# HyperBitGore/deflate.hpp

Hardware: AMD Instinct MI355X
Metric: GB/s deflate+inflate on 1 GiB buffer at 1/2/4/8 MI355X; ratio vs reference (higher is better)
Workload: dtype u8; 1 GPU; deflate level 2 + inflate round trip of a per-GPU 1 GiB 'repeat' corpus (SURVEY App. B), device-resident; corpus=repeat, bytes_per_gpu=1073741824, level=2, segment_bytes=32768, parallelism=shard1

## Files before the change

deflate.hpp_amd/csrc/deflate_kernels.hip:

```cpp
#include "dmx_device.h"
#include "dmx_internal.h"

namespace dmx {

constexpr int DF_NT = 1024;
constexpr int DF_CHUNK = 258;
constexpr int df_hash_bits(int seg) {
    return seg >= 32768 ? 12 : 11;
}
constexpr int DF_LIT_MAXBITS = 9;
constexpr int DF_DIST_MAXBITS = 6;
constexpr int DF_L3_DEPTH = 16;
constexpr uint32_t DF_L3_LONG = 16;
constexpr uint32_t DF_L3_RP = 512;
constexpr bool df_early(int seg) { return seg >= 32768; }
constexpr uint32_t EM_ALL_LITERALS = 0xFFFFFFFFu;


__device__ __forceinline__ int df_tid() {
    int t = threadIdx.x;
    asm volatile("" : "+v"(t));
    return t;
}

// ... 318 lines not shown
            const uint64_t d = *B.nseg_dev;
            return d < A.nseg ? d : A.nseg;
        }
    }
    return A.nseg;
}

template <int SEG, bool BATCH, bool DICT = false>
__device__ __forceinline__ DfSegAddr df_seg_addr(const DeflateArgs& A, uint64_t seg) {
    static_assert(!DICT || BATCH, "the dictionary comes with the batch's segment table");
    DfSegAddr s;
    s.dict = nullptr;
    s.dlen = 0;
    if constexpr (BATCH) {
        const DeflateBatchSeg e = A.btab[seg];
        s.src = e.src;
        s.tail = e.tail;
        s.nb = e.nb;
        s.is_last = (e.buf & DF_BATCH_LAST) != 0;
        if constexpr (DICT) {
            s.dict = e.dict;
            s.dlen = (uint32_t)e.dlen;
        }
    } else {
        const uint64_t base = seg * (uint64_t)SEG;
        s.src = A.in + base;
        s.tail = A.n - base;
        s.nb = (uint32_t)min((uint64_t)SEG, A.n - base);
        s.is_last = seg + 1 == A.nseg;
    }
    return s;
}

template <int SEG, bool BATCH, bool DICT = false>
__device__ __forceinline__ bool df_prefetch_next(const DeflateArgs& A, uint64_t seg, uint32_t* image) {
    bool go;
    const uint8_t* nsrc;
    if constexpr (BATCH) {
        go = seg + gridDim.x < df_nseg<true>(A);
        if (go) {
            const DeflateBatchSeg e = A.btab[seg + gridDim.x];
            nsrc = e.src;
            go = e.nb == (uint32_t)SEG && ((reinterpret_cast<uintptr_t>(nsrc) & 15) == 0);
            if constexpr (DICT) go = go && e.dlen == 0;
        } else {
            nsrc = nullptr;
        }
    } else {
        const uint64_t nbase = (seg + gridDim.x) * (uint64_t)SEG;
        nsrc = A.in + nbase;
        go = seg + gridDim.x < A.nseg && nbase + SEG <= A.n && ((reinterpret_cast<uintptr_t>(A.in + nbase) & 15) == 0);
    }
    if (go) {
        const int t = df_tid();
        const uint4* src = reinterpret_cast<const uint4*>(nsrc) + t;
        uint4* dst = reinterpret_cast<uint4*>(image) + (t & ~63);
        if constexpr (df_early(SEG)) {
            static_assert(4 * DfSmem<SEG>::NWALK <= DF_NT / 2, "the walk leaves the upper waves idle");
            if (t >= DF_NT / 2) {
                const uint32_t base = __builtin_amdgcn_readfirstlane(
                    (uint32_t)(uintptr_t)(__attribute__((address_space(3))) void*)(dst - DF_NT / 2));
#pragma unroll
                for (int k = 0; k < SEG / (8 * DF_NT); k++) {
                    uint32_t keep;
                    asm volatile("s_mov_b32 %0, m0\n\ts_mov_b32 m0, %2\n\ts_nop 0\n\t"
                                 "global_load_lds_dwordx4 %1, off\n\ts_mov_b32 m0, %0"
                                 : "=&s"(keep)
                                 : "v"(src - DF_NT / 2 + k * (DF_NT / 2)), "s"(base + (uint32_t)(k * DF_NT * 8))
                                 : "memory");
                }
            }
        } else {
#pragma unroll
            for (int k = 0; k < SEG / (16 * DF_NT); k++)
                __builtin_amdgcn_global_load_lds(src + k * DF_NT, (__attribute__((address_space(3))) void*)(dst + k * DF_NT),
                                                 16, 0, 0);
        }
    }
    return go;
}

struct TokRange {
    uint32_t w, m, n;
};
__device__ __forceinline__ uint32_t next_tok(const uint32_t* tokmap, uint32_t& w, uint32_t& m) {
    while (!m) m = tokmap[++w];
    const uint32_t p = w * 32 + __builtin_ctz(m);
    m &= m - 1;
    return p;
}

__device__ __forceinline__ void df_load_at(uint8_t* dbytes, uint32_t off, const uint8_t* src, uint32_t n, int t) {
    uint32_t head = (16u - (off & 15u)) & 15u;
    if (((reinterpret_cast<uintptr_t>(src) + head) & 15) != 0 || head > n) head = n;
    for (uint32_t i = t; i < head; i += DF_NT) dbytes[off + i] = src[i];
    const uint32_t nvec = (n - head) / 16;
    const uint4* s4 = reinterpret_cast<const uint4*>(src + head);
    uint4* d4 = reinterpret_cast<uint4*>(dbytes + off + head);
    for (uint32_t i = t; i < nvec; i += DF_NT) d4[i] = s4[i];
    for (uint32_t i = head + 16 * nvec + t; i < n; i += DF_NT) dbytes[off + i] = src[i];
}

template <int SEG, bool L3, bool BATCH, bool DICT>
__device__ __forceinline__ void deflate_segment(const DeflateArgs& A, DfSmem<SEG>& S, uint64_t seg,
                                                uint32_t& staged, [[maybe_unused]] uint32_t iw) {
    constexpr bool EARLY = DfSmem<SEG>::EARLY;
    uint32_t *data32, *U;
    if constexpr (EARLY) {
        data32 = &S.buf[0][0] + iw;
        U = &S.buf[0][0] + ((uint32_t)DfSmem<SEG>::BW - iw);
    } else {
        data32 = S.data32;
        U = S.U;
    }
    [[maybe_unused]] constexpr int NWALK = DfSmem<SEG>::NWALK;
    constexpr int HT = DfSmem<SEG>::HT;
    constexpr int NMAP = SEG / 32;
    const int t = df_tid();
    const DfSegAddr sa = df_seg_addr<SEG, BATCH, DICT>(A, seg);
    const uint32_t D = DICT ? sa.dlen : 0u;
    const uint32_t nb = D + sa.nb;
    constexpr int level = L3 ? 3 : 2;
    uint8_t* const dbytes = reinterpret_cast<uint8_t*>(data32);
    constexpr bool TERMRUN = !L3 && SEG >= 32768;
    constexpr uint32_t RUN_NONE = 0xFFFFFFFFu;
    DMX_PHASE(A.dbg, seg, 0);

    {
        const uint8_t* src = sa.src;
        const uint32_t nvec = nb / 16;
        if (staged) {
        } else if (DICT && D) {
            df_load_at(dbytes, 0, sa.dict, D, t);
            df_load_at(dbytes, D, src, nb - D, t);
        } else if ((((uintptr_t)src) & 15) == 0) {
            const uint4* s4 = reinterpret_cast<const uint4*>(src);
// ... 254 lines not shown
                    for (int j = 0; j < 4; j++) {
                        m |= ((x[j] & 0xFFFFu) ? 1u : 0u) << (8 * k + 2 * j);
                        m |= ((x[j] >> 16) ? 1u : 0u) << (8 * k + 2 * j + 1);
                    }
                }
                const uint32_t b0 = 32 * w;
                S.mmap[w] = b0 + 32 <= nb ? m : (nb > b0 ? m & ((1u << (nb - b0)) - 1u) : 0u);
            }
            if (TERMRUN && run_lo != RUN_NONE) {
                const uint32_t v = run_d | (run_d << 16);
                const uint32_t i0 = run_lo / 8, i1 = max(i0, (nb - 11) / 8 + 1);
                uint4* const c4 = reinterpret_cast<uint4*>(S.cand);
                for (uint32_t i = i0 + t; i < i1; i += DF_NT) c4[i] = make_uint4(v, v, v, v);
                const uint32_t p = 8 * i1 + t;
                if (t < 16 && p < nb) S.cand[p] = (uint16_t)(p + 4 <= nb ? run_d : 0u);
                constexpr uint32_t RP = 2 * DF_NT;
                const uint32_t bq = run_lo - RP + 4 * (uint32_t)t;
                if ((uint32_t)t < RP / 4 && bq >= run_d) {
                    const uint32_t ia = (bq - run_d) >> 2;
                    const uint32_t df = data32[bq >> 2] ^
                                        __builtin_amdgcn_alignbyte(data32[ia + 1], data32[ia], (run_lo - run_d) & 3);
                    if (df) atomicMax(&S.sh[43], ((run_lo / RP + 1) << 16) | (bq + 4 - ((uint32_t)__builtin_clz(df) >> 3)));
                }
            }
            __syncthreads();
            if (TERMRUN && run_lo != RUN_NONE) {
                constexpr uint32_t RP = 2 * DF_NT;
                const uint32_t et = __builtin_amdgcn_readfirstlane(S.sh[43]);
                run_e = (et >> 16) == run_lo / RP + 1 ? et & 0xFFFFu : max(run_lo - RP, (run_d + 3) & ~3u);
                run_rcp = __builtin_amdgcn_rcpf((float)run_d);
            }
        }
        DMX_PHASE(A.dbg, seg, 2);
        if constexpr (EARLY) staged = df_prefetch_next<SEG, BATCH, DICT>(A, seg, U);

        constexpr uint32_t CH = DF_CHUNK;
        const uint32_t nwalk = (nb - D + CH - 1) / CH;
        auto parse_walk = [&](auto runc) {
            constexpr bool RUNW = decltype(runc)::value;
            const uint32_t sub = t & 3;
            const bool lead = sub == 0;
            const uint32_t lo = D + (t >> 2) * CH;
            const uint32_t hi = min(lo + CH, nb);
            auto bits_range = [](uint32_t a, uint32_t b, uint32_t w) -> uint32_t {
                const uint32_t e = b - w * 32;
                return (e >= 32 ? 0xFFFFFFFFu : ((1u << e) - 1u)) & (0xFFFFFFFFu << (a & 31));
            };
            [[maybe_unused]] auto known_len = [&](uint32_t q, uint32_t d) -> bool {
                const uint32_t m = (uint32_t)((float)d * run_rcp + 0.5f);
                return (q >= run_e) & (m * run_d == d) & (q - d + run_d >= run_e);
            };
            auto len_at = [&](uint32_t q, uint32_t d, uint32_t maxl) -> uint32_t {
                if (!RUNW) return matchlen4(data32, q, q - d, maxl, sub);
                const bool kn = known_len(q, d);
                const uint32_t L = matchlen4(data32, q, q - d, kn ? 0u : maxl, sub);
                return kn ? maxl : L;
            };
            auto full_len = [&](uint32_t q) -> uint32_t {
                return len_at(q, S.cand[q], min(258u, hi - q));
            };
            uint32_t p = lo, w = lo >> 5, mw = S.mmap[w], tok = 0, lastp = lo;
            auto mbit = [&](uint32_t q) -> bool {
                return (S.mmap[q >> 5] >> (q & 31)) & 1u;
            };
            while (p < hi) {
                const uint32_t wi = p >> 5;
                if (wi != w) {
// ... 284 lines not shown
                    uint32_t w = tr.w, m = tr.m, lit = 0, nl = 0;
                    for (uint32_t i = 0; i < tr.n; i++) {
                        const uint32_t p = next_tok(S.tokmap, w, m);
                        const uint32_t d = S.cand[p];
                        if (d) {
                            if (nl) emit(lit | (nl << 24));
                            nl = 0;
                            lit = 0;
                            emit(0x80000000u | ((uint32_t)(S.cand[p + 1] - 3) << 16) | (d - 1));
                        } else {
                            lit |= (uint32_t)data_byte(data32, p) << (8 * nl);
                            if (++nl == 3) {
                                emit(lit | (3u << 24));
                                nl = 0;
                                lit = 0;
                            }
                        }
                    }
                    if (nl) emit(lit | (nl << 24));
                };
                uint32_t nw = 0;
                walk([&](uint32_t) { nw++; });
                uint32_t wtot;
                const uint32_t woff = block_excl_scan(nw, S.scan, &wtot);
                uint32_t* const dst = A.tok + seg * (uint64_t)A.tok_stride + woff;
                uint32_t j = 0;
                walk([&](uint32_t v) { dst[j++] = v; });
                if (t == 0) A.ntok[seg] = wtot;
            }
        }
        DMX_PHASE(A.dbg, seg, 11);
        if constexpr (!EARLY) {
            __syncthreads();
            staged = df_prefetch_next<SEG, BATCH, DICT>(A, seg, data32);
        }
        DMX_PHASE(A.dbg, seg, 10);
    }
}

template <int SEG, bool L3, bool BATCH, bool DICT>
__device__ __forceinline__ void deflate_segments(const DeflateArgs& A, DfSmem<SEG>& S) {
    constexpr bool EARLY = DfSmem<SEG>::EARLY;
    uint32_t staged = 0;
    uint32_t iw = 0;
    if constexpr (EARLY) {
        const int t = df_tid();
        if (t < 64) S.buf[t >> 5][SEG / 4 + (t & 31)] = 0;
    }
    for (uint64_t seg = blockIdx.x; seg < df_nseg<BATCH>(A); seg += gridDim.x) {
        deflate_segment<SEG, L3, BATCH, DICT>(A, S, seg, staged, iw);
        if constexpr (EARLY) {
            df_lds_barrier();
            iw = (uint32_t)DfSmem<SEG>::BW - iw;
        } else
            __syncthreads();
    }
}
template <int SEG, bool L3, bool BATCH = false, bool DICT = false>
__global__ __launch_bounds__(DF_NT) void k_deflate_segments(DeflateArgs A) {
    static_assert(!BATCH && !DICT, "a batch runs k_deflate_segments_batch");
    __shared__ DfSmem<SEG> S;
    deflate_segments<SEG, L3, false, false>(A, S);
}
template <bool L3, bool BATCH = false>
__global__ __launch_bounds__(DF_NT) __attribute__((amdgpu_waves_per_eu(8, 8))) void k_deflate_segments16(DeflateArgs A) {
    static_assert(!BATCH, "a batch runs k_deflate_segments16_batch");
    __shared__ DfSmem<16384> S;
    deflate_segments<16384, L3, false, false>(A, S);
}
template <int SEG, bool L3, bool DICT = false>
__global__ __launch_bounds__(DF_NT) void k_deflate_segments_batch(DeflateBatchArgs A) {
    __shared__ DfSmem<SEG> S;
    deflate_segments<SEG, L3, true, DICT>(A, S);
}
template <bool L3>
__global__ __launch_bounds__(DF_NT) __attribute__((amdgpu_waves_per_eu(8, 8))) void k_deflate_segments16_batch(DeflateBatchArgs A) {
    __shared__ DfSmem<16384> S;
    deflate_segments<16384, L3, true, false>(A, S);
}

constexpr int EM_NW = 4;
constexpr int EM_FLUSH = 256;
constexpr int EM_STG = 576;
constexpr int EM_LIT = 288, EM_SYM = 320;

struct EmWave {
    union {
        uint32_t freq[EM_SYM];
        uint32_t stg[EM_STG];
    };
    uint32_t code[EM_SYM];
    uint8_t len[EM_SYM];
    uint16_t rk[EM_SYM];
    uint32_t prefreq[20];
    uint32_t precode[20];
    uint8_t prelen[24];
    uint32_t hcnt[6][20];
    uint32_t lcnt[6][16];
    uint32_t kpre[2][20];
    uint32_t start[2][16];
    uint32_t next[2][16];
};

struct EmCodes {
    uint32_t dyn_tok, fix_tok;
    uint32_t nlit, ndist;
};

__device__ __forceinline__ uint32_t em_slot(int c, int lane) { return c < 5 ? 64 * c + lane : EM_LIT + lane; }
__device__ __forceinline__ bool em_valid(int c, int lane) { return c < 5 ? 64 * c + lane < 286 : lane < 30; }

__device__ EmCodes em_build_codes(EmWave& W) {
    const int lane = lane_id();
    const uint64_t lt = (1ull << lane) - 1ull;
    uint32_t Fl = 0, nzl = 0, hil = 0;
    for (int c = 0; c < 5; c++) {
        const uint32_t f = em_valid(c, lane) ? W.freq[em_slot(c, lane)] : 0u;
        Fl += f;
        const uint64_t b = __ballot(f != 0);
        nzl += (uint32_t)__popcll(b);
        if (b) hil = 64 * c + 64 - (uint32_t)__clzll(b);
    }
    Fl = wave_sum(Fl);
    const uint32_t f5 = lane < 30 ? W.freq[EM_LIT + lane] : 0u;
    const uint32_t Fd = wave_sum(f5);
    const uint64_t bd = __ballot(f5 != 0);
    const uint32_t nzd = (uint32_t)__popcll(bd), hid = bd ? 64 - (uint32_t)__clzll(bd) : 0u;
    for (int c = 0; c < 6; c++) {
        const uint32_t f = em_valid(c, lane) ? W.freq[em_slot(c, lane)] : 0u;
        const uint32_t F = c < 5 ? Fl : Fd;
        const uint32_t L0 = init_len(f, F, c < 5 ? DF_LIT_MAXBITS : DF_DIST_MAXBITS);
        const uint32_t k0 = L0 ? 2 * L0 + (((uint64_t)f << L0) <= F ? 1u : 0u) : 0u;
        uint32_t mine = 0, w0 = 0;
#pragma unroll
        for (int k = 2; k <= 2 * DF_LIT_MAXBITS + 1; k++) {
// ... 468 lines not shown
        }
        return w;
    };
#pragma unroll 4
    for (uint32_t k4 = lane; k4 < n16; k4 += 64) {
        uint4 o;
        if (const uint32_t sh = data_shift(16 * k4, 16 * k4 + 16)) {
            const uint32_t x = 16 * k4 - sh + mis, i0 = x >> 2, s = x & 3;
            const uint32_t a0 = inw[i0], a1 = inw[i0 + 1], a2 = inw[i0 + 2], a3 = inw[i0 + 3];
            const uint32_t a4 = i0 + 4 < in_words_end ? inw[i0 + 4] : 0u;
            o.x = __builtin_amdgcn_alignbyte(a1, a0, s);
            o.y = __builtin_amdgcn_alignbyte(a2, a1, s);
            o.z = __builtin_amdgcn_alignbyte(a3, a2, s);
            o.w = __builtin_amdgcn_alignbyte(a4, a3, s);
        } else {
            o.x = word_at(4 * k4);
            o.y = word_at(4 * k4 + 1);
            o.z = word_at(4 * k4 + 2);
            o.w = word_at(4 * k4 + 3);
        }
        slot4[k4] = o;
    }
    if (lane == 0) A.sizes[seg] = total;
}

template <int SEG, bool RAW, bool BATCH = false>
__global__ __launch_bounds__(64 * EM_NW) __attribute__((amdgpu_waves_per_eu(6))) void k_deflate_emit(DeflateArgs A) {
    static_assert(!BATCH, "a batch runs k_deflate_emit_batch");
    __shared__ EmWave Ws[EM_NW];
    const uint64_t seg = (uint64_t)blockIdx.x * EM_NW + (threadIdx.x >> 6);
    if (seg >= A.nseg) return;
    em_segment<SEG, RAW, false>(A, Ws[threadIdx.x >> 6], seg);
}
template <int SEG, bool RAW>
__global__ __launch_bounds__(64 * EM_NW) __attribute__((amdgpu_waves_per_eu(6))) void k_deflate_emit_batch(DeflateBatchArgs A) {
    __shared__ EmWave Ws[EM_NW];
    const uint64_t seg = (uint64_t)blockIdx.x * EM_NW + (threadIdx.x >> 6);
    if (seg >= df_nseg<true>(A)) return;
    em_segment<SEG, RAW, true>(A, Ws[threadIdx.x >> 6], seg);
}

constexpr uint32_t SCAN_NT = 256, SCAN_PER = 32, SCAN_BLK = SCAN_NT * SCAN_PER;
__device__ __forceinline__ void scan_load32(const uint32_t* v, uint64_t i, uint64_t n, bool vec, uint32_t (&x)[32]) {
    if (vec && i + 32 <= n) {
        const uint4* s4 = reinterpret_cast<const uint4*>(v + i);
#pragma unroll
        for (int k = 0; k < 8; k++) {
            const uint4 q = s4[k];
            x[4 * k] = q.x;
            x[4 * k + 1] = q.y;
            x[4 * k + 2] = q.z;
            x[4 * k + 3] = q.w;
        }
    } else {
#pragma unroll
        for (int k = 0; k < 32; k++) x[k] = i + k < n ? v[i + k] : 0u;
    }
}
__device__ __forceinline__ uint64_t scan_block64(uint64_t s, uint64_t* part, uint64_t* all) {
    const int t = threadIdx.x, lane = t & 63, wave = t >> 6;
    uint64_t inc = s;
#pragma unroll
    for (int d = 1; d < 64; d <<= 1) {
        const uint32_t lo = (uint32_t)__shfl_up((int)(uint32_t)inc, d, 64);
        const uint32_t hi = (uint32_t)__shfl_up((int)(uint32_t)(inc >> 32), d, 64);
        if (lane >= d) inc += ((uint64_t)hi << 32) | lo;
// ... 111 lines not shown
        r.path = 0;
        A.bres[b] = r;
        return;
    }
    const uint64_t s0 = A.bfirst[b], s1 = A.bfirst[b + 1];
    uint64_t bytes;
    if (s0 == s1) {
        bytes = 2;
        if (A.bcap[b] >= 2) {
            A.bout[b][0] = 0x03;
            A.bout[b][1] = 0x00;
        }
    } else {
        bytes = (s1 < A.nseg ? A.offsets[s1] : *A.total) - A.offsets[s0];
    }
    ::dmx_batch_result r;
    r.bytes = bytes;
    r.status = bytes > A.bcap[b] ? DMX_ERR_CAPACITY : DMX_OK;
    r.path = 0;
    A.bres[b] = r;
}

uint64_t deflate_front_fit(uint32_t seg_bytes) {
    int dev = 0, ncu = 0, per = 0;
    (void)hipGetDevice(&dev);
    (void)hipDeviceGetAttribute(&ncu, hipDeviceAttributeMultiprocessorCount, dev);
    if (seg_bytes >= 32768)
        (void)hipOccupancyMaxActiveBlocksPerMultiprocessor(&per, k_deflate_segments<32768, false>, DF_NT, 0);
    else
        (void)hipOccupancyMaxActiveBlocksPerMultiprocessor(&per, k_deflate_segments16<false>, DF_NT, 0);
    return (uint64_t)max(ncu, 1) * (uint64_t)max(per, 1);
}

hipError_t launch_deflate(const DeflateArgs& A, uint32_t seg_bytes, hipStream_t st,
                          hipEvent_t ev_main0, hipEvent_t ev_main1, bool dict, const uint64_t* nseg_dev,
                          const uint8_t* bflag) {
    if (dict && (!A.btab || seg_bytes != 32768)) return hipErrorInvalidValue;
    const uint64_t fit = deflate_front_fit(seg_bytes);
    const uint32_t grid = (uint32_t)std::min<uint64_t>(A.nseg, fit);
    if (ev_main0) (void)hipEventRecord(ev_main0, st);
    if (A.btab) {
        if (seg_bytes != 32768 && seg_bytes != 16384) return hipErrorInvalidValue;
        DeflateBatchArgs B;
        static_cast<DeflateArgs&>(B) = A;
        B.nseg_dev = nseg_dev;
        B.bflag = bflag;
        const bool l3 = A.level >= 3, s32 = seg_bytes == 32768;
        if (grid && A.level >= 2 && dict) {
            if (l3) hipLaunchKernelGGL((k_deflate_segments_batch<32768, true, true>), dim3(grid), dim3(DF_NT), 0, st, B);
            else hipLaunchKernelGGL((k_deflate_segments_batch<32768, false, true>), dim3(grid), dim3(DF_NT), 0, st, B);
        } else if (grid && A.level >= 2) {
            if (s32 && l3) hipLaunchKernelGGL((k_deflate_segments_batch<32768, true>), dim3(grid), dim3(DF_NT), 0, st, B);
            else if (s32) hipLaunchKernelGGL((k_deflate_segments_batch<32768, false>), dim3(grid), dim3(DF_NT), 0, st, B);
            else if (l3) hipLaunchKernelGGL((k_deflate_segments16_batch<true>), dim3(grid), dim3(DF_NT), 0, st, B);
            else hipLaunchKernelGGL((k_deflate_segments16_batch<false>), dim3(grid), dim3(DF_NT), 0, st, B);
        }
        if (A.nseg) {
            const uint32_t eg = (uint32_t)((A.nseg + EM_NW - 1) / EM_NW);
            const bool raw = A.level < 2;
            if (s32 && raw) hipLaunchKernelGGL((k_deflate_emit_batch<32768, true>), dim3(eg), dim3(64 * EM_NW), 0, st, B);
            else if (s32) hipLaunchKernelGGL((k_deflate_emit_batch<32768, false>), dim3(eg), dim3(64 * EM_NW), 0, st, B);
            else if (raw) hipLaunchKernelGGL((k_deflate_emit_batch<16384, true>), dim3(eg), dim3(64 * EM_NW), 0, st, B);
            else hipLaunchKernelGGL((k_deflate_emit_batch<16384, false>), dim3(eg), dim3(64 * EM_NW), 0, st, B);
        }
        if (ev_main1) (void)hipEventRecord(ev_main1, st);
        const hipError_t e = launch_scan_u32(A.sizes, A.offsets, A.nseg, A.total, st);
        if (e != hipSuccess) return e;
        const uint64_t waves = A.nseg + (A.nbuf + 63) / 64;
        hipLaunchKernelGGL(k_compact_batch, dim3((uint32_t)((waves + 3) / 4)), dim3(256), 0, st, B);
        return hipGetLastError();
    }
    if (grid && A.level >= 2) {
        const bool l3 = A.level >= 3;
// ... 51 lines not shown
```

deflate.hpp_amd/csrc/dmx_ctx.h:

```cpp
#pragma once
#include <hip/hip_runtime.h>

#include <mutex>
#include <string>
#include <vector>

#include "../../include/dmx.h"
#include "dmx_internal.h"

namespace dmx {

struct DevBuf {
    void* p = nullptr;
    size_t cap = 0;
    bool ensure(size_t bytes) {
        if (bytes <= cap) return true;
        if (p) (void)hipFree(p);
        p = nullptr;
        cap = 0;
        size_t want = bytes + bytes / 8 + 4096;
        if (hipMalloc(&p, want) != hipSuccess) {
            p = nullptr;
            return false;
        }
// ... 17 lines not shown
    uint32_t seg = 32768;
    uint32_t flags = 0;
    int inflate_pass = -1;
    uint32_t heavy_bytes = 0;
    uint32_t diag = 0;
    hipStream_t stream = nullptr;
    std::mutex mu;
    DevBuf in, out, slots, sizes, offs, scal, cands, tiles, tileoffs, recs, status, dbg;
    DevBuf dtok, dntok;
    DevBuf rtmp, rchain;
    DevBuf ltok, ltokoff, lntok, lcaps, lsplit;
    DevBuf lheavy;
    int ncu = 256;
    DevBuf fbc, fbh, fbo, fbl, fbs, fbt, fbk, fbu, fbch, fbco, fbcs, fbimg, fbstop, fbwin, fbopen;
    DevBuf fbvm, fbvh;
    DevBuf fbph;
    uint64_t* fbkeep_h = nullptr;
    uint64_t* fbkeep_d = nullptr;
    uint8_t* pin = nullptr;
    size_t pin_cap = 0, pin_off = 0;
    DevBuf fbreg, fbJ, fbvis;
    DevBuf fbJraw, fbJsub, fbcbit, fbucb;
    DevBuf ck;
    DevBuf btab, bres;
    DevBuf adf, ainf;
    DevBuf fdesc;
    DevBuf bgzs, bgzc, bgzd, bgzt;
    bool timing = false;
    hipEvent_t ev[4] = {nullptr, nullptr, nullptr, nullptr};
    hipEvent_t ev_df = nullptr;
    hipEvent_t ev_inf = nullptr;
    bool inf_pending = false;
    bool df_pending = false;
    dmx_stats stats{};
    uint64_t last_end = 0;
    std::vector<dmx_ctx*> subs;
};

namespace dmx {

enum : uint32_t { DIAG_PHASES = 1, DIAG_FB = 2, DIAG_RECS = 4, DIAG_DEBUG = 8, DIAG_FBT = 16 };
struct Diag {
    uint32_t bits = 0;
    std::string phases_path;
};
const Diag& diag_env();
void hipchk_report(const char* what, hipError_t e, const char* file, int line);
#define HIPCHK(x)                                          \
    do {                                                   \
        const hipError_t e_ = (x);                         \
        if (e_ != hipSuccess) {                            \
            hipchk_report(#x, e_, __FILE_NAME__, __LINE__); \
            return DMX_ERR_DEVICE;                         \
        }                                                  \
    } while (0)

struct Scal {
    uint64_t total;
    uint64_t nmarkers;
    uint32_t ticket;
    uint32_t fb_err;
    uint32_t fb_nkeep;
    uint64_t ncand;
    InflateResult res;
    ValidateWords vw;
};
// ... 25 lines not shown
```

deflate.hpp_amd/csrc/dmx_host.cpp:

```cpp
#include <hip/hip_runtime.h>

#include <algorithm>
#include <condition_variable>
#include <cstdio>
#include <thread>
#include <cstdlib>
#include <vector>
#include <cstring>
#include <mutex>
#include <new>
#include <string>

#include "dmx_ctx.h"

using namespace dmx;

namespace dmx {

const Diag& diag_env() {
    static const Diag d = [] {
        Diag r;
        if (std::getenv("DMX_DEBUG")) r.bits |= DIAG_DEBUG;
        if (const char* e = std::getenv("DMX_PHASES")) r.bits |= DIAG_PHASES, r.phases_path = e;
        if (const char* e = std::getenv("DMX_FB_DEBUG"); e && *e) r.bits |= DIAG_FB;
// ... 83 lines not shown
void end_timing(dmx_ctx* c, hipStream_t st) {
    if (!c->timing) return;
    (void)hipEventRecord(c->ev[3], st);
    (void)hipEventSynchronize(c->ev[3]);
    float a = 0, b = 0;
    (void)hipEventElapsedTime(&a, c->ev[0], c->ev[3]);
    (void)hipEventElapsedTime(&b, c->ev[1], c->ev[2]);
    (void)hipGetLastError();
    c->stats.ms_device_total = a;
    c->stats.ms_main_kernel = b;
}

}

namespace {

bool deflate_scratch(dmx_ctx* c, DeflateArgs& A, uint64_t nseg, uint64_t nfront, int level, uint32_t fseg_bytes) {
    const uint64_t ns = std::max<uint64_t>(1, nseg), nf = std::max<uint64_t>(1, nfront);
    A.nseg = nseg;
    A.level = level;
    A.slot_bytes = c->seg + 256;
    A.tok_stride = level >= 2 ? deflate_tok_stride(fseg_bytes) : 0u;
    if (!c->slots.ensure(ns * (size_t)A.slot_bytes) || !c->sizes.ensure(ns * 4) || !c->offs.ensure(scan_words(nseg) * 8) ||
        !c->dtok.ensure(std::max<uint64_t>(1, nfront * (uint64_t)A.tok_stride) * 4) || !c->dntok.ensure(nf * 4))
        return false;
    A.slots = c->slots.as<uint8_t>();
    A.tok = c->dtok.as<uint32_t>();
    A.ntok = c->dntok.as<uint32_t>();
    A.sizes = c->sizes.as<uint32_t>();
    A.offsets = c->offs.as<uint64_t>();
    return true;
}

int deflate_device_locked(dmx_ctx* c, const uint8_t* d_in, size_t n, int level, uint32_t flags,
                          uint8_t* d_out, size_t cap, size_t* out_len, hipStream_t st,
                          uint64_t* d_total = nullptr) {
    if (level < 0 || level > 3) level = 1;
    const bool final_last = (flags & DMX_DEFLATE_NOT_FINAL) == 0;
    const bool async = d_total != nullptr;
    if (c->df_pending) HIPCHK(hipStreamWaitEvent(st, c->ev_df, 0));
    if (!async) begin_timing(c, st);
    if (n == 0) {
        static const uint8_t empty_final[2] = {0x03, 0x00};
        static const uint64_t lens[2] = {0, 2};
        if (out_len) *out_len = final_last ? 2 : 0;
        if (async) {
            if (final_last && cap >= 2) HIPCHK(hipMemcpyAsync(d_out, empty_final, 2, hipMemcpyHostToDevice, st));
            HIPCHK(hipMemcpyAsync(d_total, &lens[final_last ? 1 : 0], 8, hipMemcpyHostToDevice, st));
            return DMX_OK;
        }
        if (!final_last) return DMX_OK;
        if (cap < 2) return DMX_ERR_CAPACITY;
        HIPCHK(hipMemcpyAsync(d_out, empty_final, 2, hipMemcpyHostToDevice, st));
        HIPCHK(hipStreamSynchronize(st));
        return DMX_OK;
    }
    const uint64_t nseg = (n + c->seg - 1) / c->seg;
    const uint32_t fseg_bytes = std::min<uint32_t>(c->seg, 32768);
    DeflateArgs A;
    if (!c->scal.ensure(sizeof(Scal)) || !deflate_scratch(c, A, nseg, (n + fseg_bytes - 1) / fseg_bytes, level, fseg_bytes))
        return DMX_ERR_NOMEM;
    A.in = d_in;
    A.n = n;
    A.final_last = final_last ? 1 : 0;
    A.total = async ? d_total : &c->scal.as<Scal>()->total;
    A.out = d_out;
    A.cap = cap;
    A.dbg = async ? nullptr : phase_buf(c, nseg);
    const bool tm = c->timing && !async;
    HIPCHK(launch_deflate(A, c->seg, st, tm ? c->ev[1] : nullptr, tm ? c->ev[2] : nullptr));
    HIPCHK(hipEventRecord(c->ev_df, st));
    c->df_pending = true;
    if (async) return DMX_OK;
    if (A.dbg) phase_dump(c, "deflate", nseg, st, c->seg == 65536 ? 0 : std::min<uint64_t>(nseg, deflate_front_fit(c->seg)));
    uint64_t total = 0;
    HIPCHK(hipMemcpyAsync(&total, A.total, 8, hipMemcpyDeviceToHost, st));
    HIPCHK(hipStreamSynchronize(st));
    end_timing(c, st);
    c->stats.segments = nseg;
    c->stats.in_bytes = n;
    c->stats.out_bytes = total;
    *out_len = total;
    return total > cap ? DMX_ERR_CAPACITY : DMX_OK;
}


struct FramePlan {
    uint32_t format;
    int level;
    bool verify;
    const InflateBatchDesc* hdesc;
};
int checksum_locked(dmx_ctx* c, bool crc, const uint8_t* d, size_t n, uint32_t init, uint32_t* out, hipStream_t st);

int deflate_batch_locked(dmx_ctx* c, const uint8_t* const* d_in, const size_t* n, size_t count, int level,
                         uint8_t* const* d_out, const size_t* cap, dmx_batch_result* res, hipStream_t st,
                         const uint8_t* d_dict = nullptr, size_t dict_len = 0, const FramePlan* fp = nullptr) {
    if (level < 0 || level > 3) level = 1;
    const uint32_t seg = c->seg;
    const uint32_t du = level >= 2 ? (uint32_t)std::min<size_t>(dict_len, kDeflateDictMax) : 0u;
    if (du && seg != 32768) return DMX_ERR_ARG;
    const uint8_t* const dtail = du ? d_dict + (dict_len - du) : nullptr;
    const size_t seg0 = seg - du;
// ... 518 lines not shown

void dmx_config_default(dmx_config* cfg) {
    cfg->device = -1;
    cfg->segment_bytes = 32768;
    cfg->flags = 0;
    cfg->n_gpus = 1;
    cfg->dev_inflate_pass = 0;
    cfg->dev_heavy_bytes = 0;
}

int dmx_create(dmx_ctx** out, const dmx_config* cfg) {
    if (!out) return DMX_ERR_ARG;
    *out = nullptr;
    dmx_config d;
    dmx_config_default(&d);
    if (!cfg) cfg = &d;
    if (cfg->segment_bytes != 16384 && cfg->segment_bytes != 32768 && cfg->segment_bytes != 65536) return DMX_ERR_ARG;
    int ndev = 0;
    if (hipGetDeviceCount(&ndev) != hipSuccess || ndev <= 0) return DMX_ERR_DEVICE;
    int dev = cfg->device;
    if (dev < 0 && hipGetDevice(&dev) != hipSuccess) return DMX_ERR_DEVICE;
    if (dev >= ndev || !is_gfx950(dev)) return DMX_ERR_DEVICE;
    if (cfg->n_gpus > 8u * (uint32_t)ndev) return DMX_ERR_ARG;
    DeviceGuard dg(dev);
    if (!dg.ok) return DMX_ERR_DEVICE;
    dmx_ctx* c = new (std::nothrow) dmx_ctx();
    if (!c) return DMX_ERR_NOMEM;
    c->device = dev;
    c->seg = cfg->segment_bytes;
    c->flags = cfg->flags;
    c->inflate_pass = (int)cfg->dev_inflate_pass - 1;
    c->heavy_bytes = cfg->dev_heavy_bytes;
    c->diag = diag_env().bits;
    if (hipDeviceGetAttribute(&c->ncu, hipDeviceAttributeMultiprocessorCount, dev) != hipSuccess || c->ncu <= 0)
        c->ncu = 256;
    if (hipStreamCreateWithFlags(&c->stream, hipStreamNonBlocking) != hipSuccess) {
        delete c;
        return DMX_ERR_DEVICE;
    }
    for (auto& e : c->ev) (void)hipEventCreate(&e);
    if (hipEventCreateWithFlags(&c->ev_df, hipEventDisableTiming) != hipSuccess ||
        hipEventCreateWithFlags(&c->ev_inf, hipEventDisableTiming) != hipSuccess) {
        dmx_destroy(c);
        return DMX_ERR_DEVICE;
    }
    if (cfg->n_gpus > 1) {
        dmx_config sc = *cfg;
        sc.n_gpus = 1;
        for (uint32_t i = 0; i < cfg->n_gpus; i++) {
            sc.device = (dev + (int)i) % ndev;
            dmx_ctx* s = nullptr;
            const int rc = is_gfx950(sc.device) ? dmx_create(&s, &sc) : DMX_ERR_DEVICE;
            if (rc != DMX_OK) {
                dmx_destroy(c);
                return rc;
            }
            c->subs.push_back(s);
        }
    }
    *out = c;
    return DMX_OK;
}

void dmx_destroy(dmx_ctx* c) {
    if (!c) return;
    for (dmx_ctx* s : c->subs) dmx_destroy(s);
    c->subs.clear();
    DeviceGuard dg(c->device);
    (void)hipStreamSynchronize(c->stream);
    if (c->df_pending && c->ev_df) (void)hipEventSynchronize(c->ev_df);
    if (c->inf_pending && c->ev_inf) (void)hipEventSynchronize(c->ev_inf);
    for (DevBuf* b : {&c->in, &c->out, &c->slots, &c->sizes, &c->offs, &c->scal, &c->cands,
                      &c->tiles, &c->tileoffs, &c->recs, &c->status, &c->dbg, &c->ltok,
                      &c->ltokoff, &c->lntok, &c->lcaps, &c->lheavy, &c->rtmp, &c->rchain, &c->fbc, &c->fbh, &c->fbo, &c->fbl,
                      &c->fbs, &c->fbt, &c->fbk, &c->fbu, &c->fbch, &c->fbco, &c->fbcs, &c->fbimg, &c->fbstop, &c->fbwin, &c->fbopen, &c->fbvm, &c->fbvh,
                      &c->fbreg, &c->fbJ, &c->fbvis, &c->fbph,
                      &c->ck, &c->btab, &c->bres, &c->adf, &c->ainf, &c->fdesc, &c->bgzs, &c->bgzc, &c->bgzd, &c->bgzt})
        b->release();
    for (auto& e : c->ev)
        if (e) (void)hipEventDestroy(e);
    if (c->ev_df) (void)hipEventDestroy(c->ev_df);
    if (c->ev_inf) (void)hipEventDestroy(c->ev_inf);
    if (c->fbkeep_h) (void)hipHostFree(c->fbkeep_h);
    if (c->pin) (void)hipHostFree(c->pin);
    (void)hipStreamDestroy(c->stream);
    delete c;
}

static std::mutex g_default_mu;
static dmx_config g_default_cfg;
static bool g_default_set = false, g_default_made = false;

int dmx_set_default_config(const dmx_config* cfg) {
    if (!cfg) return DMX_ERR_ARG;
    std::lock_guard<std::mutex> g(g_default_mu);
    if (g_default_made) return DMX_ERR_ARG;
    g_default_cfg = *cfg;
    g_default_set = true;
    return DMX_OK;
}

dmx_ctx* dmx_default_ctx(void) {
    static std::once_flag once;
    static dmx_ctx* ctx = nullptr;
    std::call_once(once, [] {
        std::lock_guard<std::mutex> g(g_default_mu);
        g_default_made = true;
        if (dmx_create(&ctx, g_default_set ? &g_default_cfg : nullptr) != DMX_OK) ctx = nullptr;
    });
    return ctx;
}

size_t dmx_deflate_bound(size_t n) { return n + 10 * ((n + 16383) / 16384) + 16; }

int dmx_deflate_device(dmx_ctx* c, const void* d_in, size_t n, int level, uint32_t flags,
// ... 1275 lines not shown
```

deflate.hpp_amd/csrc/dmx_internal.h:

```cpp
#pragma once
#include <hip/hip_runtime.h>
#include <stdint.h>

#include "../../include/dmx.h"
#include "container_parse.h"
#include "bgzf_chain.h"
#include "batch_table.h"
#include "inflate_records.h"

namespace dmx {

constexpr uint32_t kDeflateDictMax = 16384;
constexpr uint32_t kInflateDictMax = 32768;

struct DeflateArgs {
    const uint8_t* in;
    uint64_t n;
    uint64_t nseg;
    int level;
    int final_last;
    uint8_t* slots;
    uint32_t slot_bytes;
    uint32_t* tok;
    uint32_t tok_stride;
    uint32_t* ntok;
    uint32_t* sizes;
    uint64_t* offsets;
    uint64_t* total;
    uint8_t* out;
    uint64_t cap;
    uint64_t* dbg;
    const DeflateBatchSeg* btab = nullptr;
    const uint64_t* bfirst = nullptr;
    uint8_t* const* bout = nullptr;
    const uint64_t* bcap = nullptr;
    ::dmx_batch_result* bres = nullptr;
    uint64_t nbuf = 0;
};
struct DeflateBatchArgs : DeflateArgs {
    const uint64_t* nseg_dev = nullptr;
    const uint8_t* bflag = nullptr;
};

constexpr uint32_t deflate_tok_stride(uint32_t seg) { return seg / 2 + 1248; }
static_assert(deflate_tok_stride(32768) == 17632 && deflate_tok_stride(16384) == 9440,
              "the token buffers' layout is fixed");

hipError_t launch_deflate(const DeflateArgs& A, uint32_t seg_bytes, hipStream_t st, hipEvent_t ev0,
                          hipEvent_t ev1, bool dict = false, const uint64_t* nseg_dev = nullptr,
                          const uint8_t* bflag = nullptr);
uint64_t deflate_front_fit(uint32_t seg_bytes);

constexpr uint32_t DMX_IFLAG_PIECE = 1u << 31;

struct InflateArgs {
    const uint32_t* in_words;
    uint64_t misalign;
    uint64_t n;
    const uint64_t* cands;
    uint64_t ncand;
    uint8_t* out;
    uint64_t cap;
    SegRecord* recs;
    unsigned long long* status;
    unsigned int* ticket;
    uint32_t flags;
    uint32_t mode;
    uint32_t slot;
    uint64_t* dbg;
    const uint64_t* ncand_dev = nullptr;
};
__device__ __forceinline__ uint64_t cand_count(const InflateArgs& A) {
    return A.ncand_dev ? (*A.ncand_dev < A.ncand ? *A.ncand_dev : A.ncand) : A.ncand;
}

constexpr int kPhaseSlots = 16;
#define DMX_PHASE(dbg, idx, slot)                                                   \
    do {                                                                            \
        if ((dbg) && threadIdx.x == 0) (dbg)[(idx) * kPhaseSlots + (slot)] = __builtin_amdgcn_s_memtime(); \
    } while (0)

struct InflateResult {
    uint64_t total;
// ... 134 lines not shown
```

Measured before the change: 428.9 GB/s.

## Pipeline deflate front and emission stages across chunks on a side stream

Splits the segment range into a few chunks (four by default) and launches the front parse kernel per chunk on the main stream. Each chunk's emission kernel runs on a low-priority side stream, gated by events, so emission of chunk i overlaps the front pass of chunk i+1. The goal is to hide the serial front-then-emit gap and fill idle CUs, relying on emission waves fitting beside a front workgroup's LDS. The cost is extra launches, event syncs and a side stream, plus possible contention or tail imbalance between the two kernels.

```diff
diff --git a/deflate.hpp_amd/csrc/deflate_kernels.hip b/deflate.hpp_amd/csrc/deflate_kernels.hip
--- a/deflate.hpp_amd/csrc/deflate_kernels.hip
+++ b/deflate.hpp_amd/csrc/deflate_kernels.hip
@@ -374,8 +374,9 @@
     return s;
 }
 
-template <int SEG, bool BATCH, bool DICT = false>
+template <int SEG, bool BATCH, bool DICT = false, bool PIPE = false>
 __device__ __forceinline__ bool df_prefetch_next(const DeflateArgs& A, uint64_t seg, uint32_t* image) {
+    static_assert(!PIPE || !BATCH, "the chunk pipeline is the single-stream path's");
     bool go;
     const uint8_t* nsrc;
     if constexpr (BATCH) {
@@ -391,7 +392,9 @@
     } else {
         const uint64_t nbase = (seg + gridDim.x) * (uint64_t)SEG;
         nsrc = A.in + nbase;
-        go = seg + gridDim.x < A.nseg && nbase + SEG <= A.n && ((reinterpret_cast<uintptr_t>(A.in + nbase) & 15) == 0);
+        uint64_t end = A.nseg;
+        if constexpr (PIPE) end = static_cast<const DeflatePipeArgs&>(A).seg_end;
+        go = seg + gridDim.x < end && nbase + SEG <= A.n && ((reinterpret_cast<uintptr_t>(A.in + nbase) & 15) == 0);
     }
     if (go) {
         const int t = df_tid();
@@ -443,7 +446,7 @@
     for (uint32_t i = head + 16 * nvec + t; i < n; i += DF_NT) dbytes[off + i] = src[i];
 }
 
-template <int SEG, bool L3, bool BATCH, bool DICT>
+template <int SEG, bool L3, bool BATCH, bool DICT, bool PIPE = false>
 __device__ __forceinline__ void deflate_segment(const DeflateArgs& A, DfSmem<SEG>& S, uint64_t seg,
                                                 uint32_t& staged, [[maybe_unused]] uint32_t iw) {
     constexpr bool EARLY = DfSmem<SEG>::EARLY;
@@ -764,7 +767,7 @@
             }
         }
         DMX_PHASE(A.dbg, seg, 2);
-        if constexpr (EARLY) staged = df_prefetch_next<SEG, BATCH, DICT>(A, seg, U);
+        if constexpr (EARLY) staged = df_prefetch_next<SEG, BATCH, DICT, PIPE>(A, seg, U);
 
         constexpr uint32_t CH = DF_CHUNK;
         const uint32_t nwalk = (nb - D + CH - 1) / CH;
@@ -1115,13 +1118,13 @@
         DMX_PHASE(A.dbg, seg, 11);
         if constexpr (!EARLY) {
             __syncthreads();
-            staged = df_prefetch_next<SEG, BATCH, DICT>(A, seg, data32);
+            staged = df_prefetch_next<SEG, BATCH, DICT, PIPE>(A, seg, data32);
         }
         DMX_PHASE(A.dbg, seg, 10);
     }
 }
 
-template <int SEG, bool L3, bool BATCH, bool DICT>
+template <int SEG, bool L3, bool BATCH, bool DICT, bool PIPE = false>
 __device__ __forceinline__ void deflate_segments(const DeflateArgs& A, DfSmem<SEG>& S) {
     constexpr bool EARLY = DfSmem<SEG>::EARLY;
     uint32_t staged = 0;
@@ -1130,8 +1133,14 @@
         const int t = df_tid();
         if (t < 64) S.buf[t >> 5][SEG / 4 + (t & 31)] = 0;
     }
-    for (uint64_t seg = blockIdx.x; seg < df_nseg<BATCH>(A); seg += gridDim.x) {
-        deflate_segment<SEG, L3, BATCH, DICT>(A, S, seg, staged, iw);
+    uint64_t first = 0;
+    if constexpr (PIPE) first = static_cast<const DeflatePipeArgs&>(A).seg_first;
+    const auto end = [&]() -> uint64_t {
+        if constexpr (PIPE) return static_cast<const DeflatePipeArgs&>(A).seg_end;
+        else return df_nseg<BATCH>(A);
+    };
+    for (uint64_t seg = first + blockIdx.x; seg < end(); seg += gridDim.x) {
+        deflate_segment<SEG, L3, BATCH, DICT, PIPE>(A, S, seg, staged, iw);
         if constexpr (EARLY) {
             df_lds_barrier();
             iw = (uint32_t)DfSmem<SEG>::BW - iw;
@@ -1160,6 +1169,11 @@
 __global__ __launch_bounds__(DF_NT) __attribute__((amdgpu_waves_per_eu(8, 8))) void k_deflate_segments16_batch(DeflateBatchArgs A) {
     __shared__ DfSmem<16384> S;
     deflate_segments<16384, L3, true, false>(A, S);
+}
+template <bool L3>
+__global__ __launch_bounds__(DF_NT) __attribute__((amdgpu_num_vgpr(52))) void k_deflate_segments_pipe(DeflatePipeArgs A) {
+    __shared__ DfSmem<32768> S;
+    deflate_segments<32768, L3, false, false, true>(A, S);
 }
 
 constexpr int EM_NW = 4;
@@ -1184,6 +1198,7 @@
     uint32_t start[2][16];
     uint32_t next[2][16];
 };
+static_assert(3 * sizeof(EmWave) <= 163840 - 140320, "three emission waves fit beside a front workgroup's LDS");
 
 struct EmCodes {
     uint32_t dyn_tok, fix_tok;
@@ -1718,6 +1733,13 @@
     if (seg >= A.nseg) return;
     em_segment<SEG, RAW, false>(A, Ws[threadIdx.x >> 6], seg);
 }
+template <int SEG, int NW>
+__global__ __launch_bounds__(64 * NW) __attribute__((amdgpu_waves_per_eu(6))) void k_deflate_emit_pipe(DeflatePipeArgs A) {
+    __shared__ EmWave Ws[NW];
+    const uint64_t seg = A.seg_first + (uint64_t)blockIdx.x * NW + (threadIdx.x >> 6);
+    if (seg >= A.seg_end) return;
+    em_segment<SEG, false, false>(A, Ws[threadIdx.x >> 6], seg);
+}
 template <int SEG, bool RAW>
 __global__ __launch_bounds__(64 * EM_NW) __attribute__((amdgpu_waves_per_eu(6))) void k_deflate_emit_batch(DeflateBatchArgs A) {
     __shared__ EmWave Ws[EM_NW];
@@ -1895,13 +1917,60 @@
     return (uint64_t)max(ncu, 1) * (uint64_t)max(per, 1);
 }
 
+static hipError_t launch_deflate_pipe(const DeflateArgs& A, uint32_t seg_bytes, hipStream_t st, const DeflatePipe& P) {
+    const uint32_t halves = seg_bytes == 65536 ? 2 : 1;
+    const uint64_t nfront = seg_bytes == 65536 ? (A.n + 32767) / 32768 : A.nseg;
+    const uint64_t fit = deflate_front_fit(32768);
+    const uint64_t nchunk = pipe_chunk_count(A.nseg, P.chunk);
+    DeflatePipeArgs F, E;
+    static_cast<DeflateArgs&>(F) = A;
+    static_cast<DeflateArgs&>(E) = A;
+    F.nseg = nfront;
+    F.dbg = nullptr;
+    for (uint64_t i = 0; i < nchunk; i++) {
+        const PipeRange r = pipe_range(A.nseg, P.chunk, i), f = pipe_front_range(r, halves, nfront);
+        F.seg_first = f.first, F.seg_end = f.end;
+        E.seg_first = r.first, E.seg_end = r.end;
+        const uint32_t grid = (uint32_t)std::min<uint64_t>(f.end - f.first, fit);
+        if (grid) {
+            if (A.level >= 3) hipLaunchKernelGGL(k_deflate_segments_pipe<true>, dim3(grid), dim3(DF_NT), 0, st, F);
+            else hipLaunchKernelGGL(k_deflate_segments_pipe<false>, dim3(grid), dim3(DF_NT), 0, st, F);
+        }
+        const bool last = i + 1 == nchunk;
+        if (!last) {
+            hipError_t e = hipEventRecord(P.ev_chunk, st);
+            if (e == hipSuccess) e = hipStreamWaitEvent(P.side, P.ev_chunk, 0);
+            if (e != hipSuccess) return e;
+        }
+        const hipStream_t es = last ? st : P.side;
+        const uint64_t ne = r.end - r.first;
+        if (halves == 2) hipLaunchKernelGGL((k_deflate_emit_pipe<65536, 1>), dim3((uint32_t)ne), dim3(64), 0, es, E);
+        else hipLaunchKernelGGL((k_deflate_emit_pipe<32768, 1>), dim3((uint32_t)ne), dim3(64), 0, es, E);
+    }
+    hipError_t e = hipEventRecord(P.ev_side, P.side);
+    if (e == hipSuccess) e = hipStreamWaitEvent(st, P.ev_side, 0);
+    return e != hipSuccess ? e : hipGetLastError();
+}
+
 hipError_t launch_deflate(const DeflateArgs& A, uint32_t seg_bytes, hipStream_t st,
                           hipEvent_t ev_main0, hipEvent_t ev_main1, bool dict, const uint64_t* nseg_dev,
-                          const uint8_t* bflag) {
+                          const uint8_t* bflag, const DeflatePipe* pipe) {
     if (dict && (!A.btab || seg_bytes != 32768)) return hipErrorInvalidValue;
+    if (pipe && (A.btab || A.level < 2 || seg_bytes < 32768 || A.dbg || !pipe->chunk || pipe->chunk >= A.nseg))
+        return hipErrorInvalidValue;
     const uint64_t fit = deflate_front_fit(seg_bytes);
     const uint32_t grid = (uint32_t)std::min<uint64_t>(A.nseg, fit);
     if (ev_main0) (void)hipEventRecord(ev_main0, st);
+    if (pipe) {
+        hipError_t e = launch_deflate_pipe(A, seg_bytes, st, *pipe);
+        if (e != hipSuccess) return e;
+        if (ev_main1) (void)hipEventRecord(ev_main1, st);
+        e = launch_scan_u32(A.sizes, A.offsets, A.nseg, A.total, st);
+        if (e != hipSuccess) return e;
+        hipLaunchKernelGGL(k_compact, dim3((uint32_t)((A.nseg + 3) / 4)), dim3(256), 0, st, A.slots, A.slot_bytes,
+                           A.sizes, A.offsets, A.nseg, A.out, A.cap);
+        return hipGetLastError();
+    }
     if (A.btab) {
         if (seg_bytes != 32768 && seg_bytes != 16384) return hipErrorInvalidValue;
         DeflateBatchArgs B;
diff --git a/deflate.hpp_amd/csrc/deflate_pipe.h b/deflate.hpp_amd/csrc/deflate_pipe.h
--- /dev/null
+++ b/deflate.hpp_amd/csrc/deflate_pipe.h
@@ -0,0 +1,58 @@
+#pragma once
+#include <stdint.h>
+
+namespace dmx {
+
+struct PipeRange {
+    uint64_t first, end;
+};
+
+inline uint64_t pipe_chunk_segs(uint64_t nseg, uint64_t fit, uint32_t chunks, uint64_t forced) {
+    if (forced) return nseg > forced ? forced : 0;
+    if (fit == 0 || chunks < 2 || nseg < 2 * fit) return 0;
+    const uint64_t per = (nseg + chunks - 1) / chunks;
+    const uint64_t c = (per + fit - 1) / fit * fit;
+    return c < nseg ? c : 0;
+}
+inline uint64_t pipe_chunk_count(uint64_t nseg, uint64_t chunk) { return (nseg + chunk - 1) / chunk; }
+inline PipeRange pipe_range(uint64_t nseg, uint64_t chunk, uint64_t i) {
+    const uint64_t a = i * chunk, b = a + chunk;
+    return {a, b < nseg ? b : nseg};
+}
+inline PipeRange pipe_front_range(PipeRange r, uint32_t halves, uint64_t nfront) {
+    const uint64_t a = r.first * halves, b = r.end * halves;
+    return {a < nfront ? a : nfront, b < nfront ? b : nfront};
+}
+
+struct PipeKnob {
+    bool on;
+    bool explicit_on;
+    uint32_t chunks;
+    uint64_t forced;
+};
+constexpr bool kPipeDefaultOn = true;
+constexpr uint32_t kPipeDefaultChunks = 4;
+inline PipeKnob pipe_knob(const char* e) {
+    PipeKnob k{kPipeDefaultOn, false, kPipeDefaultChunks, 0};
+    if (!e || !*e) return k;
+    const bool seg = *e == 's';
+    uint64_t v = 0;
+    const char* p = e + (seg ? 1 : 0);
+    if (!*p) return k;
+    for (; *p; p++) {
+        if (*p < '0' || *p > '9' || v > (1u << 24)) return k;
+        v = v * 10 + (uint64_t)(*p - '0');
+    }
+    if (seg) {
+        if (v) k.on = k.explicit_on = true, k.forced = v;
+    } else if (v == 0) {
+        k.on = false;
+    } else if (v == 1) {
+        k.on = k.explicit_on = true;
+    } else if (v <= 64) {
+        k.on = k.explicit_on = true, k.chunks = (uint32_t)v;
+    }
+    return k;
+}
+
+}
diff --git a/deflate.hpp_amd/csrc/dmx_ctx.h b/deflate.hpp_amd/csrc/dmx_ctx.h
--- a/deflate.hpp_amd/csrc/dmx_ctx.h
+++ b/deflate.hpp_amd/csrc/dmx_ctx.h
@@ -73,6 +73,9 @@
     hipEvent_t ev_inf = nullptr;
     bool inf_pending = false;
     bool df_pending = false;
+    dmx::PipeKnob pipe{};
+    hipStream_t side = nullptr;
+    hipEvent_t ev_chunk = nullptr, ev_side = nullptr;
     dmx_stats stats{};
     uint64_t last_end = 0;
     std::vector<dmx_ctx*> subs;
diff --git a/deflate.hpp_amd/csrc/dmx_host.cpp b/deflate.hpp_amd/csrc/dmx_host.cpp
--- a/deflate.hpp_amd/csrc/dmx_host.cpp
+++ b/deflate.hpp_amd/csrc/dmx_host.cpp
@@ -139,6 +139,24 @@
     return true;
 }
 
+bool pipe_streams(dmx_ctx* c) {
+    if (c->side) return true;
+    int lo = 0, hi = 0;
+    (void)hipDeviceGetStreamPriorityRange(&lo, &hi);
+    if (hipStreamCreateWithPriority(&c->side, hipStreamNonBlocking, lo) != hipSuccess) {
+        c->side = nullptr;
+        return false;
+    }
+    if (hipEventCreateWithFlags(&c->ev_chunk, hipEventDisableTiming) != hipSuccess ||
+        hipEventCreateWithFlags(&c->ev_side, hipEventDisableTiming) != hipSuccess) {
+        if (c->ev_chunk) (void)hipEventDestroy(c->ev_chunk);
+        (void)hipStreamDestroy(c->side);
+        c->side = nullptr, c->ev_chunk = c->ev_side = nullptr;
+        return false;
+    }
+    return true;
+}
+
 int deflate_device_locked(dmx_ctx* c, const uint8_t* d_in, size_t n, int level, uint32_t flags,
                           uint8_t* d_out, size_t cap, size_t* out_len, hipStream_t st,
                           uint64_t* d_total = nullptr) {
@@ -175,7 +193,15 @@
     A.cap = cap;
     A.dbg = async ? nullptr : phase_buf(c, nseg);
     const bool tm = c->timing && !async;
-    HIPCHK(launch_deflate(A, c->seg, st, tm ? c->ev[1] : nullptr, tm ? c->ev[2] : nullptr));
+    DeflatePipe P{0, nullptr, nullptr, nullptr};
+    if (c->pipe.on && level >= 2 && !A.dbg &&
+        (c->pipe.explicit_on ? c->seg >= 32768 : c->seg == 32768 && !async)) {
+        P.chunk = pipe_chunk_segs(nseg, deflate_front_fit(c->seg), c->pipe.chunks, c->pipe.forced);
+        if (P.chunk && !pipe_streams(c)) return DMX_ERR_DEVICE;
+        P.side = c->side, P.ev_chunk = c->ev_chunk, P.ev_side = c->ev_side;
+    }
+    HIPCHK(launch_deflate(A, c->seg, st, tm ? c->ev[1] : nullptr, tm ? c->ev[2] : nullptr, false, nullptr, nullptr,
+                          P.chunk ? &P : nullptr));
     HIPCHK(hipEventRecord(c->ev_df, st));
     c->df_pending = true;
     if (async) return DMX_OK;
@@ -760,6 +786,7 @@
     c->inflate_pass = (int)cfg->dev_inflate_pass - 1;
     c->heavy_bytes = cfg->dev_heavy_bytes;
     c->diag = diag_env().bits;
+    c->pipe = pipe_knob(std::getenv("DMX_DEFLATE_PIPE"));
     if (hipDeviceGetAttribute(&c->ncu, hipDeviceAttributeMultiprocessorCount, dev) != hipSuccess || c->ncu <= 0)
         c->ncu = 256;
     if (hipStreamCreateWithFlags(&c->stream, hipStreamNonBlocking) != hipSuccess) {
@@ -809,6 +836,12 @@
         if (e) (void)hipEventDestroy(e);
     if (c->ev_df) (void)hipEventDestroy(c->ev_df);
     if (c->ev_inf) (void)hipEventDestroy(c->ev_inf);
+    if (c->side) {
+        (void)hipStreamSynchronize(c->side);
+        (void)hipStreamDestroy(c->side);
+        (void)hipEventDestroy(c->ev_chunk);
+        (void)hipEventDestroy(c->ev_side);
+    }
     if (c->fbkeep_h) (void)hipHostFree(c->fbkeep_h);
     if (c->pin) (void)hipHostFree(c->pin);
     (void)hipStreamDestroy(c->stream);
diff --git a/deflate.hpp_amd/csrc/dmx_internal.h b/deflate.hpp_amd/csrc/dmx_internal.h
--- a/deflate.hpp_amd/csrc/dmx_internal.h
+++ b/deflate.hpp_amd/csrc/dmx_internal.h
@@ -6,6 +6,7 @@
 #include "container_parse.h"
 #include "bgzf_chain.h"
 #include "batch_table.h"
+#include "deflate_pipe.h"
 #include "inflate_records.h"
 
 namespace dmx {
@@ -41,6 +42,14 @@
     const uint64_t* nseg_dev = nullptr;
     const uint8_t* bflag = nullptr;
 };
+struct DeflatePipeArgs : DeflateArgs {
+    uint64_t seg_first = 0, seg_end = 0;
+};
+struct DeflatePipe {
+    uint64_t chunk;
+    hipStream_t side;
+    hipEvent_t ev_chunk, ev_side;
+};
 
 constexpr uint32_t deflate_tok_stride(uint32_t seg) { return seg / 2 + 1248; }
 static_assert(deflate_tok_stride(32768) == 17632 && deflate_tok_stride(16384) == 9440,
@@ -48,7 +57,7 @@
 
 hipError_t launch_deflate(const DeflateArgs& A, uint32_t seg_bytes, hipStream_t st, hipEvent_t ev0,
                           hipEvent_t ev1, bool dict = false, const uint64_t* nseg_dev = nullptr,
-                          const uint8_t* bflag = nullptr);
+                          const uint8_t* bflag = nullptr, const DeflatePipe* pipe = nullptr);
 uint64_t deflate_front_fit(uint32_t seg_bytes);
 
 constexpr uint32_t DMX_IFLAG_PIECE = 1u << 31;
```

Result: faster. 439.4 GB/s (median of 6 runs) (+2.5%).
